# isabella232/kyverno

Measured on AMD Instinct MI355X. Metric: resource×rule validate evals/sec (node), higher is better.
Workload: dtype u8; 1 GPU; C2: synthetic Pods x 100 validate.pattern rules (image globs, ?*, quantities, |-lists); rules=100, pairs_per_gpu=100000000, output=full, parallelism=resource-shard x1, engine=specialized

## Files before the change

### kyverno_amd/csrc/kvapi.cpp

```cpp
#include <hip/hip_runtime.h>
#include <rccl/rccl.h>

#include <chrono>
#include <cstdio>
#include <cstring>

#define KVRT_DEVICE 1
#include "kvrt.hpp"
#include "kvdev.h"

namespace kvh {

struct DevPolicySet {
  DevBuf prog, preds, alts, conjs, atoms, rules, filters, kinds, strrefs, strpairs, sels, sellabels, selexprs, kgs,
      gsegs, gwords, pstr, fword, fbit, flist, frule, rcompact, gsdesc, gsmem;
  uint32_t gs_groups = 0, gs_members = 0;
  DevPS view{};
  std::vector<hipModule_t> mods;
  std::vector<hipFunction_t> fns;
  std::map<uint32_t, std::vector<hipFunction_t>> vfns;
  const std::vector<hipFunction_t>& fns_for(uint32_t full) const {
    auto it = vfns.find(full);
    return it == vfns.end() ? fns : it->second;
  }
// ... 94 lines not shown
    for (const JitImage::Variant& v : J.variants) {
      std::map<std::string, hipFunction_t> vname;
      for (size_t i = 0; i < v.codes.size() && i < J.kernel_name.size(); i++) {
        if (v.codes[i].empty()) continue;
        hipModule_t m;
        HIPCHK(hipModuleLoadData(&m, v.codes[i].data()));
        d->mods.push_back(m);
        hipFunction_t f;
        HIPCHK(hipModuleGetFunction(&f, m, J.kernel_name[i].c_str()));
        vname[J.kernel_name[i]] = f;
      }
      std::vector<hipFunction_t>& fv = d->vfns[v.full];
      for (auto& ch : J.chunks) {
        auto it = vname.find(ch.name);
        fv.push_back(it != vname.end() ? it->second : byname.at(ch.name));
      }
    }
    for (auto& ch : J.chunks) {
      auto it = byname.find(ch.name);
      if (it == byname.end()) throw std::runtime_error("specialized kernel " + ch.name + " missing");
      hipFunction_t f = it->second;
      d->fns.push_back(f);
      if (getenv("KVGPU_VERBOSE")) {
        int regs = 0, local = 0;
        (void)hipFuncGetAttribute(&regs, HIP_FUNC_ATTRIBUTE_NUM_REGS, f);
        (void)hipFuncGetAttribute(&local, HIP_FUNC_ATTRIBUTE_LOCAL_SIZE_BYTES, f);
        fprintf(stderr, "[kvgpu] %s: %zu rules, %d VGPRs, %d B scratch/lane\n", ch.name.c_str(), ch.rules.size(), regs,
                local);
      }
    }
    d->rcompact.upload(J.rec_compact, device);
    if (!J.gs_desc.empty()) {
      d->gs_groups = (uint32_t)(J.gs_desc.size() / 4u);
      d->gs_members = J.gs_members;
      d->gsdesc.upload(J.gs_desc, device);
      d->gsmem.upload(J.gs_mem, device);
    }
    if (J.mtup_words) {
      d->mtup_words = J.mtup_words;
      d->fac_slots = J.fac_slots;
      d->fword.upload(J.fac_word, device);
      d->fbit.upload(J.fac_bit, device);
      d->flist.upload(J.fac_flist, device);
      d->frule.upload(J.fac_rule, device);
      v.fac_word = (const uint32_t*)d->fword.p;
      v.fac_bit = (const uint32_t*)d->fbit.p;
      v.fac_flist = (const uint32_t*)d->flist.p;
      v.fac_rule = (const uint32_t*)d->frule.p;
      v.fac_slots = J.fac_slots;
      v.fac_words = J.mtup_words;
    }
    if (J.memo_words) {
      d->ptab_fn = byname.at("kvj_ptab");
      d->memo_words = J.memo_words;
      d->ptab_rows = (uint32_t)((J.memo_preds.size() + J.ptab_row - 1) / J.ptab_row);
    }
  }
  auto& ref = *d;
  s->dev[device] = std::move(d);
  return ref;
}

void build_pcol(const JitImage& J, const Batch& b, DevBatchRes* d, int device) {
  const auto t0 = std::chrono::steady_clock::now();
  const uint32_t nf = (uint32_t)J.fam_ncols.size(), j0 = J.fam_ncols.at(0);
  const uint64_t groups64 = (b.res.size() + KV_WG - 1) / KV_WG * (KV_WG / KV_LANES);
  if (groups64 > 0x3FFFFFFull) throw std::runtime_error("path columns: too many resources");
  const uint32_t groups = (uint32_t)groups64;
  d->pcold.upload(J.cols, device);
  d->perow.alloc((size_t)std::max<uint32_t>(1u, nf - 1) * (groups + 1) * sizeof(uint32_t), device);
  HIPCHK(hipMemset(d->perow.p, 0, d->perow.n));
  std::vector<ColFam> fams(nf);
  uint32_t n_wide = 0, n_narrow = 0;
  for (uint32_t f = 0; f < nf; f++) {
    fams[f].arr_col = J.fam_arr[f];
    fams[f].ncols = J.fam_ncols[f];
    fams[f].nw = J.fam_nw.at(f);
    fams[f].nb = J.fam_nb.at(f);
    fams[f].nn = J.fam_nn.at(f);
    fams[f].erow = f ? (uint32_t*)d->perow.p + (size_t)(f - 1) * (groups + 1) : nullptr;
    n_wide += fams[f].nw;
    n_narrow += fams[f].nn;
  }
  if (n_narrow && b.vals.size() + KV_PTAB_PSEUDO >= (1ull << KV_COL_PAYLOAD))
    throw std::runtime_error("path columns: more than 2^28 distinct values");
  d->pfam.upload(fams, device);
  const DevBatch* Bd = (const DevBatch*)d->view_dev.p;
  const ColDesc* cd = (const ColDesc*)d->pcold.p;
  std::vector<uint32_t> erow;
  if (nf > 1) {
    HIPCHK(launch_pcol_rows(Bd, cd, (const ColFam*)d->pfam.p, nf, groups, nullptr));
    erow.resize((size_t)(nf - 1) * (groups + 1));
    HIPCHK(hipMemcpy(erow.data(), d->perow.p, erow.size() * sizeof(uint32_t), hipMemcpyDeviceToHost));
  }
  auto row_words = [&](uint32_t f) { return (uint64_t)(3u * fams[f].nw + fams[f].nb + fams[f].nn) * KV_LANES; };
  const uint64_t root_words = (uint64_t)groups * row_words(0);
  uint64_t words = root_words;
  for (uint32_t f = 1; f < nf; f++) {
    fams[f].off_lo = (uint32_t)words;
    fams[f].off_hi = (uint32_t)(words >> 32);
    words += (uint64_t)erow[(size_t)(f - 1) * (groups + 1) + groups] * row_words(f);
  }
  if (words >= (1ull << 32)) throw std::runtime_error("path columns: more than 2^32 words");
  HIPCHK(hipMemcpy(d->pfam.p, fams.data(), fams.size() * sizeof(ColFam), hipMemcpyHostToDevice));
  d->pcol.alloc(std::max<uint64_t>(words, 1) * sizeof(uint32_t), device);
  uint32_t* pool = (uint32_t*)d->pcol.p;
  if (words > root_words) HIPCHK(hipMemset(pool + root_words, 0, (words - root_words) * sizeof(uint32_t)));
  HIPCHK(launch_pcol_build(Bd, cd, (const ColFam*)d->pfam.p, 0, j0, groups, false, pool, nullptr));
  HIPCHK(launch_pcol_build(Bd, cd, (const ColFam*)d->pfam.p, j0, (uint32_t)J.cols.size() - j0, groups, true, pool,
                           nullptr));
  HIPCHK(hipStreamSynchronize(nullptr));
  d->view.pcol = pool;
  d->pcol_ms = std::chrono::duration<double, std::milli>(std::chrono::steady_clock::now() - t0).count();
  if (getenv("KVGPU_VERBOSE"))
    fprintf(stderr,
            "[kvgpu] path columns: %u wide + %u narrow columns in %u families, %llu bytes (%.1f per resource), built in "
            "%.2f ms\n",
            n_wide, n_narrow, nf, (unsigned long long)(words * sizeof(uint32_t)),
            b.res.empty() ? 0.0 : (double)(words * sizeof(uint32_t)) / (double)b.res.size(), d->pcol_ms);
}

std::shared_ptr<DevBatchRes> dev_batch(kv_batch* bt, const PolicySet& ps, int device) {
  std::lock_guard<std::mutex> g(bt->mu);
  auto it = bt->dev.find(device);
  if (it != bt->dev.end()) return it->second;
  auto d = std::make_shared<DevBatchRes>();
  const Batch& b = bt->b;
  if (b.rmask.size() != b.n_rows || b.rwide.size() != b.n_rows || b.roff.size() != b.n_rows)
    throw std::runtime_error("batch: packed row arrays do not match the row count");
  hipStream_t us = StreamPool::get().take(device, hipStreamNonBlocking);
  DevBuf pc, rm, rw, ro;
  pc.upload_async(b.tcells, device, us);
  rm.upload_async(b.rmask, device, us);
  rw.upload_async(b.rwide, device, us);
  ro.upload_async(b.roff, device, us);
  d->vals.upload_async(b.vals, device, us);
  d->nodes.alloc(b.n_cells() * sizeof(Node), device);
  HIPCHK(launch_expand_rows((const uint64_t*)pc.p, (const uint64_t*)rm.p, (const uint64_t*)rw.p, (const uint32_t*)ro.p,
                            (const Val*)d->vals.p, b.n_rows, (Node*)d->nodes.p, us));
  d->res.upload_async(b.res, device, us);
  d->kvs.upload(b.kvs, device);
  d->bstr.upload_raw(b.strs.data(), b.strs.size(), device);
  d->nsbits.upload(b.ns_bits, device);
  std::vector<uint32_t> off, len;
  std::string ks;
  key_table(ps, b, &off, &len, &ks);
  d->koff.upload(off, device);
  d->klen.upload(len, device);
  d->kstr.upload_raw(ks.data(), ks.size(), device);
  d->nsms.upload(b.nsms, device);
  d->lsets.upload(b.lsets, device);
  d->asets.upload(b.asets, device);
  d->tuprep.upload(b.tup_rep, device);
  d->tupkent.upload(b.tup_kent, device);
  d->kentrep.upload(b.kent_rep, device);
  DevBatch& v = d->view;
  v.nodes = (const Node*)d->nodes.p;
  v.vals = (const Val*)d->vals.p;
  v.res = (const Res*)d->res.p;
  v.kvs = (const KV*)d->kvs.p;
  v.bstr = (const uint8_t*)d->bstr.p;
  v.ns_bits = (const uint32_t*)d->nsbits.p;
  v.key_off = (const uint32_t*)d->koff.p;
  v.key_len = (const uint32_t*)d->klen.p;
  v.kstr = (const uint8_t*)d->kstr.p;
  v.nsms = (const StrRef*)d->nsms.p;
  v.lsets = (const KVSet*)d->lsets.p;
  v.asets = (const KVSet*)d->asets.p;
  v.n_nsm = (uint32_t)b.nsms.size();
  v.n_lsets = (uint32_t)b.lsets.size();
  v.n_asets = (uint32_t)b.asets.size();
  v.ns_words = b.ns_words;
  v.n_res = (uint32_t)b.res.size();
  v.tup_rep = (const uint32_t*)d->tuprep.p;
  v.n_tup = (uint32_t)b.tup_rep.size();
  v.tup_kent = (const uint32_t*)d->tupkent.p;
  v.kent_rep = (const uint32_t*)d->kentrep.p;
  v.n_kent = (uint32_t)b.kent_rep.size();
  v.n_ns = (uint32_t)b.namespaces.size();
  {
    const DynHost& h = bt->dyn_host(ps);
    d->dpreds.upload(h.tbl.preds, device);
    d->dalts.upload(h.tbl.alts, device);
    d->dconjs.upload(h.tbl.conjs, device);
    d->datoms.upload(h.tbl.atoms, device);
    d->dgsegs.upload(h.tbl.gsegs, device);
    d->dgwords.upload(h.tbl.gwords, device);
    d->dpstr.upload_raw(h.tbl.strs.data(), h.tbl.strs.size(), device);
    DevPS dv{};
    dv.preds = (const Pred*)d->dpreds.p;
    dv.alts = (const Alt*)d->dalts.p;
    dv.conjs = (const Conj*)d->dconjs.p;
    dv.atoms = (const Atom*)d->datoms.p;
    dv.gsegs = (const GSeg*)d->dgsegs.p;
    dv.gwords = (const GWord*)d->dgwords.p;
    dv.pstr = (const uint8_t*)d->dpstr.p;
    d->dps.upload_raw(&dv, sizeof(DevPS), device);
    d->dleaf.upload(h.dleaf, device);
    d->dynst.upload(h.dyn_st, device);
    v.dps = (const DevPS*)d->dps.p;
    v.dleaf = (const uint32_t*)d->dleaf.p;
    v.dyn_st = (const uint8_t*)d->dynst.p;
  }
  auto up = [&](DevBuf* bufs, std::initializer_list<const std::vector<uint32_t>*> src, const uint32_t** dp) {
    for (const std::vector<uint32_t>* v : src) {
      bufs->alloc(std::max<size_t>(v->size() * sizeof(uint32_t), 16), device);
      if (!v->empty()) HIPCHK(hipMemcpyAsync(bufs->p, v->data(), v->size() * sizeof(uint32_t), hipMemcpyHostToDevice, us));
      *dp++ = (const uint32_t*)(bufs++)->p;
    }
  };
  auto up_blocks = [&](DevBuf* bufs, const CondHost& h, bool strict) {
    const uint32_t* dp[7] = {};
    up(bufs, {&h.sets, &h.ents, &h.outc, &h.truth, &h.unk}, dp);
    if (strict) up(bufs + 5, {&h.err, &h.oos}, dp + 5);
    return CondBlocks{dp[0], dp[1], dp[2], dp[3], dp[4], dp[5], dp[6], h.words};
  };
  struct Timed {
    hipEvent_t e0, e1;
    double* ms;
  };
  std::vector<Timed> timed;
  auto timed_launch = [&](double* ms, auto&& launch) {
    Timed t{nullptr, nullptr, ms};
    HIPCHK(hipEventCreate(&t.e0));
    HIPCHK(hipEventCreate(&t.e1));
    HIPCHK(hipEventRecord(t.e0, us));
    HIPCHK(launch());
    HIPCHK(hipEventRecord(t.e1, us));
    timed.push_back(t);
  };
  CondHost pre, dn;
  FeHost fh;
  CondBlocks pt{}, dt{};
  FeTables ft{};
  const uint32_t n_sets = (uint32_t)ps.csets.size(), n_dsets = (uint32_t)ps.dsets.size(),
                 n_fsets = (uint32_t)ps.fsets.size();
  if (n_sets && !b.res.empty()) {
    build_pre(ps, b, &pre);
    pt = up_blocks(d->pre, pre, false);
    d->prest.alloc((size_t)n_sets * b.res.size(), device);
    v.pre_st = (const uint8_t*)d->prest.p;
  }
  if (n_dsets && !b.res.empty()) {
    build_deny(ps, b, &dn);
    dt = up_blocks(d->dn, dn, true);
  }
  if (n_fsets && !b.res.empty()) {
    build_foreach(ps, b, &fh);
    const uint32_t *dp[5], *gp[2];
    up(d->fe, {&fh.sets, &fh.lists}, dp);
    up(d->feg, {&fh.gate.sets, &fh.gate.ents}, gp);
    ft = fh.view();
    ft.gate = ft.deny = up_blocks(d->fed, fh.deny, true);
    ft.gate.sets = gp[0]; ft.gate.ents = gp[1];
    up(d->fe + 2, {&fh.el_res, &fh.el_ord, &fh.lstate}, dp + 2);
    ft.sets = dp[0]; ft.lists = dp[1]; ft.el_res = dp[2]; ft.el_ord = dp[3]; ft.lstate = dp[4];
    d->feacc.alloc((size_t)n_fsets * b.res.size() * sizeof(uint32_t), device);
  }
  if ((n_dsets || n_fsets) && !b.res.empty()) {
    d->dnst.alloc((size_t)(n_dsets + n_fsets) * b.res.size(), device);
    v.deny_st = (const uint8_t*)d->dnst.p;
  }
  d->view_dev.upload_raw(&d->view, sizeof(DevBatch), device);
  if (v.pre_st) timed_launch(&d->pre_ms, [&]() { return launch_cond(false, pt, v.n_res, n_sets, (uint8_t*)d->prest.p, us); });
  if (v.deny_st && n_dsets)
    timed_launch(&d->deny_ms, [&]() { return launch_cond(true, dt, v.n_res, n_dsets, (uint8_t*)d->dnst.p, us); });
  if (v.deny_st && n_fsets)
    timed_launch(&d->fe_ms, [&]() {
      return launch_foreach(ft, v.n_res, (uint32_t*)d->feacc.p, (uint8_t*)d->dnst.p + (size_t)n_dsets * v.n_res, us);
    });
  HIPCHK(hipStreamSynchronize(us));
  for (const Timed& t : timed) {
    float ms = 0;
    HIPCHK(hipEventElapsedTime(&ms, t.e0, t.e1));
    *t.ms = ms;
    (void)hipEventDestroy(t.e0);
    (void)hipEventDestroy(t.e1);
  }
  StreamPool::get().give(device, hipStreamNonBlocking, us);
  pc.release();
  rm.release();
  rw.release();
  ro.release();
  if (bt->owner && bt->owner->jit && !bt->owner->jit->cols.empty() && !b.res.empty()) {
    build_pcol(*bt->owner->jit, b, d.get(), device);
    d->view_dev.upload_raw(&d->view, sizeof(DevBatch), device);
  }
  bt->dev[device] = d;
  return d;
}

struct DevSession {
  kv_policyset* ps = nullptr;
  kv_batch* bt = nullptr;
  int device = 0;
  uint32_t mode = 0;
  uint64_t nrules = 0, nres = 0;
  DevBuf fflags, pview, st, er8, er, cn, scope, scn, ptab, mtab, mtbf, mtup, ftab;
  DevBuf ptab1, pview1, mtab1, mtup1, ftab1, cn1, scn1;
  uint32_t *mt1_ns = nullptr, *mt1_ann = nullptr, *mt1_sel = nullptr;
  hipStream_t pside = nullptr;
  hipEvent_t ev_pt[2] = {nullptr, nullptr}, ev_rk[2] = {nullptr, nullptr};
  bool ptab_pipe = false;
  uint32_t fac_entities = 0, ntup = 0;
  bool rec_compact = false;
  std::shared_ptr<DevBatchRes> batch_ref;
  DevBuf r_offs, r_tot, r_base, r_out8, r_outw, r_wide;
  DevBuf r_tkey, r_raw, r_nbase, r_code, r_out8b;
  DevBuf s_ccnt, s_cbase, s_pack;
  HostArray<uint8_t> hstage;
  DevBuf inv_d, stc;
  DevBuf ord_d, r_mask;
  DevBuf stamps;
  DevBuf gsite, gcnt;
  DevBuf sflag;
  uint32_t mt_words = 0, mt_entities = 0;
  uint32_t *mt_ns = nullptr, *mt_ann = nullptr, *mt_sel = nullptr;
  uint32_t nscopes = 0, nvals = 0;
  DevOut O{};
  const DevBatch* bview = nullptr;
  const DevBatch* bhost = nullptr;
  DevPolicySet* dps = nullptr;
  hipStream_t stream = nullptr;
  hipEvent_t e0 = nullptr, e1 = nullptr;
  hipStream_t side = nullptr;
  hipEvent_t ev_fork = nullptr, ev_join = nullptr;
  hipEvent_t ev_rkf = nullptr, ev_rkj[3] = {};
  std::vector<hipStream_t> rkx;
  std::vector<hipEvent_t> kev;
  std::vector<uint32_t> korder;
  bool ktiming = false;

  double upload_ms = 0;
  DevSession(kv_policyset* p, kv_batch* b, const char* ctx_json, int dev, uint32_t m)
      : ps(p), bt(b), device(dev), mode(m) {
    HIPCHK(hipSetDevice(device));
    const auto tc0 = std::chrono::steady_clock::now();
    DevPolicySet& dp = dev_ps(ps, device);
    batch_ref = dev_batch(bt, ps->ps, device);
    DevBatchRes& db = *batch_ref;
    upload_ms = std::chrono::duration<double, std::milli>(std::chrono::steady_clock::now() - tc0).count();
    if (getenv("KVGPU_VERBOSE")) fprintf(stderr, "[kvgpu] session: policy set + batch upload %.1f ms\n", upload_ms);
    bview = (const DevBatch*)db.view_dev.p;
    bhost = &db.view;
    dps = &dp;
    fflags.upload(fold_filters(ps->ps, ctx_json), device);
    DevPS P = dp.view;
    P.fflags = (const uint32_t*)fflags.p;
    if (dp.ptab_fn) {
      nvals = (uint32_t)bt->b.vals.size();
      ptab.alloc((size_t)dp.memo_words * (nvals + KV_PTAB_PSEUDO) * sizeof(uint32_t), device);
      P.ptab = (const uint32_t*)ptab.p;
      P.n_vals = nvals + KV_PTAB_PSEUDO;
    }
    {
      const PolicySet& pp = ps->ps;
      const Batch& bb = bt->b;
      P.mt_ns_words = (pp.n_nss_bits + 31) / 32;
      P.mt_ann_words = (pp.n_ann_bits + 31) / 32;
      P.mt_sel_words = (uint32_t)((pp.selectors.size() + 31) / 32);
      const size_t n_ns = (size_t)P.mt_ns_words * bb.nsms.size(), n_an = (size_t)P.mt_ann_words * bb.asets.size(),
                   n_sl = (size_t)P.mt_sel_words * bb.lsets.size();
      mtab.alloc(std::max<size_t>(n_ns + n_an + n_sl, 1) * sizeof(uint32_t), device);
      mt_ns = (uint32_t*)mtab.p;
      mt_ann = mt_ns + n_ns;
      mt_sel = mt_ann + n_an;
      P.mt_ns = mt_ns;
      P.mt_ann = mt_ann;
      mtbf.upload(mtab_bit_filters(pp), device);
      P.mt_bitf = (const uint32_t*)mtbf.p;
      P.mt_sel = mt_sel;
      mt_words = P.mt_ns_words + P.mt_ann_words + P.mt_sel_words;
      mt_entities = (uint32_t)std::max({bb.nsms.size(), bb.asets.size(), bb.lsets.size()});
    }
    if (dp.mtup_words) {
      mtup.alloc(std::max<size_t>((size_t)dp.mtup_words * bt->b.tup_rep.size(), 1) * sizeof(uint32_t), device);
      P.mtup = (const uint32_t*)mtup.p;
      P.mtup_words = dp.mtup_words;
      const DevBatch& bv = *bhost;
      const uint32_t ne[KV_FAC_TYPES] = {bv.n_kent, bv.n_nsm, bv.n_asets, bv.n_lsets, bv.n_ns};
      uint64_t at = 0;
      for (uint32_t t = 0; t < KV_FAC_TYPES; t++) {
        P.fac_off[t] = at;
        at += (uint64_t)dp.fac_slots * ne[t];
        fac_entities = std::max(fac_entities, ne[t]);
      }
      ftab.alloc(std::max<uint64_t>(at, 1) * sizeof(uint32_t), device);
      P.fac_tab = (uint32_t*)ftab.p;
    }
    pview.upload_raw(&P, sizeof(DevPS), device);
    ptab_pipe = dp.specialized() && !(getenv("KVGPU_PTAB_PIPE") && getenv("KVGPU_PTAB_PIPE")[0] == '0');
    if (ptab_pipe) {
      if (dp.ptab_fn) {
        ptab1.alloc(ptab.n, device);
        P.ptab = (const uint32_t*)ptab1.p;
      }
      mtab1.alloc(mtab.n, device);
      mt1_ns = (uint32_t*)mtab1.p;
      mt1_ann = mt1_ns + (mt_ann - mt_ns);
      mt1_sel = mt1_ns + (mt_sel - mt_ns);
      P.mt_ns = mt1_ns;
      P.mt_ann = mt1_ann;
      P.mt_sel = mt1_sel;
      if (dp.mtup_words) {
        mtup1.alloc(mtup.n, device);
        P.mtup = (const uint32_t*)mtup1.p;
        ftab1.alloc(ftab.n, device);
        P.fac_tab = (uint32_t*)ftab1.p;
      }
      pview1.upload_raw(&P, sizeof(DevPS), device);
    }
    nrules = ps->ps.rules.size();
    nres = bt->b.res.size();
    ntup = (uint32_t)bt->b.tup_rep.size();
    O.full = 0;
    if ((mode & (KV_MODE_STATUS | KV_MODE_ERRORS)) || ((mode & KV_MODE_SCOPES) && !dp.specialized())) {
      st.alloc(nrules * nres, device);
      O.status = (uint8_t*)st.p;
      O.full |= 1;
      if (dp.specialized()) {
        sflag.alloc(std::max<uint64_t>(nrules * ((nres + KV_RWG - 1) / KV_RWG), 1), device);
        HIPCHK(hipMemset(sflag.p, 1, sflag.n));
        O.sflag = (uint8_t*)sflag.p;
      }
    }
    if (mode & KV_MODE_ERRORS) {
      er8.alloc(nrules * nres * sizeof(ErrRec8), device);
      O.err8 = (ErrRec8*)er8.p;
      O.err = nullptr;
      O.full |= 2;
      if (dp.gs_groups) {
        const uint64_t nw = (nres + 63) / 64;
        gsite.alloc(std::max<uint64_t>((uint64_t)dp.gs_members * nw * 64u * 16u, 16), device);
        gcnt.alloc(std::max<uint64_t>((uint64_t)dp.gs_groups * nw * sizeof(uint32_t), 4), device);
        O.gsite = (uint32_t*)gsite.p;
        O.gcnt = (uint32_t*)gcnt.p;
      }
    }
    cn.alloc(std::max<uint64_t>(nrules, 1) * KV_HIST * sizeof(unsigned long long), device);
    O.counts = (unsigned long long*)cn.p;
    if (ptab_pipe) cn1.alloc(cn.n, device);
    if (mode & KV_MODE_SCOPES) {
      std::vector<uint32_t> sc(nres);
      for (uint64_t i = 0; i < nres; i++) sc[i] = bt->b.res[i].ns_index;
      nscopes = (uint32_t)bt->b.namespaces.size();
      scope.upload(sc, device);
      scn.alloc(std::max<uint64_t>((uint64_t)nscopes * nrules, 1) * KV_HIST * sizeof(unsigned long long), device);
      if (ptab_pipe) scn1.alloc(scn.n, device);
      O.scope = (const uint32_t*)scope.p;
      O.scounts = (unsigned long long*)scn.p;
      if (dp.specialized()) O.full |= 8;
    }
    if (getenv("KVGPU_JIT_STAMPS") && dp.specialized()) {
      const uint64_t n = (nres + KV_RWG - 1) / KV_RWG * KV_RWAVES * kJitStamps;
      stamps.alloc(std::max<uint64_t>(n, 1) * sizeof(unsigned long long), device);
      HIPCHK(hipMemset(stamps.p, 0, stamps.n));
      for (hipModule_t m : dp.mods) {
        hipDeviceptr_t g = nullptr;
        size_t gs = 0;
        if (hipModuleGetGlobal(&g, &gs, m, "kvj_stamps") == hipSuccess && gs == sizeof(void*))
          HIPCHK(hipMemcpy(g, &stamps.p, sizeof(void*), hipMemcpyHostToDevice));
        else
          (void)hipGetLastError();
      }
    }
    stream = StreamPool::get().take(device, hipStreamDefault);
    HIPCHK(hipEventCreate(&e0));
    HIPCHK(hipEventCreate(&e1));
    side = StreamPool::get().take(device, hipStreamNonBlocking);
    if (ptab_pipe) {
      pside = StreamPool::get().take(device, hipStreamNonBlocking, true);
      for (int b = 0; b < 2; b++) {
        HIPCHK(hipEventCreateWithFlags(&ev_pt[b], hipEventDisableTiming));
        HIPCHK(hipEventCreateWithFlags(&ev_rk[b], hipEventDisableTiming));
      }
    }
    HIPCHK(hipEventCreateWithFlags(&ev_fork, hipEventDisableTiming));
    HIPCHK(hipEventCreateWithFlags(&ev_join, hipEventDisableTiming));
    HIPCHK(hipEventCreateWithFlags(&ev_rkf, hipEventDisableTiming));
    for (hipEvent_t& e : ev_rkj) HIPCHK(hipEventCreateWithFlags(&e, hipEventDisableTiming));
  }
  void detach_batch() { bt = nullptr; }
  void remap_scopes(const std::vector<uint32_t>& map, uint32_t n_total) {
    if (!(mode & KV_MODE_SCOPES)) return;
    HIPCHK(hipSetDevice(device));
    DevBuf m;
    m.upload(map, device);
    HIPCHK(launch_remap_u32((uint32_t*)scope.p, nres, (const uint32_t*)m.p, stream));
    HIPCHK(hipStreamSynchronize(stream));
    nscopes = n_total;
    scn.alloc(std::max<uint64_t>((uint64_t)nscopes * nrules, 1) * KV_HIST * sizeof(unsigned long long), device);
    if (ptab_pipe) scn1.alloc(scn.n, device);
    O.scounts = (unsigned long long*)scn.p;
  }
  ~DevSession() {
    (void)hipSetDevice(device);
    if (e0) (void)hipEventDestroy(e0);
    if (e1) (void)hipEventDestroy(e1);
    if (ev_fork) (void)hipEventDestroy(ev_fork);
    if (ev_join) (void)hipEventDestroy(ev_join);
    if (ev_rkf) (void)hipEventDestroy(ev_rkf);
    for (hipEvent_t e : ev_rkj)
      if (e) (void)hipEventDestroy(e);
    for (hipEvent_t e : kev) (void)hipEventDestroy(e);
    for (hipStream_t x : rkx) StreamPool::get().give(device, hipStreamNonBlocking, x);
    for (int b = 0; b < 2; b++) {
      if (ev_pt[b]) (void)hipEventDestroy(ev_pt[b]);
      if (ev_rk[b]) (void)hipEventDestroy(ev_rk[b]);
    }
    StreamPool::get().give(device, hipStreamNonBlocking, pside, true);
    StreamPool::get().give(device, hipStreamNonBlocking, side);
    StreamPool::get().give(device, hipStreamDefault, stream);
  }
  double run(int iters, bool vm = false) {
    HIPCHK(hipSetDevice(device));
    HIPCHK(hipEventRecord(e0, stream));
    const bool pipe = ptab_pipe && dps->specialized() && !vm && nres;
    if (pipe && iters > 0) {
      HIPCHK(hipStreamWaitEvent(pside, e0, 0));
      launch_tables(0);
    }
    for (int i = 0; i < iters; i++) {
      rec_compact = dps->specialized() && !vm;
      if (pipe) {
        const int b = i & 1;
        launch_specialized(b);
        if (O.full & 8u)
          HIPCHK(launch_scope_totals((const unsigned long long*)(b ? scn1.p : scn.p), nscopes, (uint32_t)nrules,
                                     (unsigned long long*)(b ? cn1.p : cn.p), stream));
        HIPCHK(hipEventRecord(ev_rk[b], stream));
        if (i + 1 < iters) {
          const int nb = (i + 1) & 1;
          if (i >= 1) HIPCHK(hipStreamWaitEvent(pside, ev_rk[nb], 0));
          launch_tables(nb);
        }
        continue;
      }
      hipStream_t ms = rec_compact ? side : stream;
      if (rec_compact) {
        HIPCHK(hipEventRecord(ev_fork, stream));
        HIPCHK(hipStreamWaitEvent(side, ev_fork, 0));
      }
      HIPCHK(hipMemsetAsync(cn.p, 0, cn.n, ms));
      if (mode & KV_MODE_SCOPES) HIPCHK(hipMemsetAsync(scn.p, 0, scn.n, ms));
      HIPCHK(launch_mtab((const DevPS*)pview.p, bview, mt_words, mt_entities, mt_ns, mt_ann, mt_sel, ms));
      if (rec_compact) {
        launch_specialized();
        if (O.full & 8u)
          HIPCHK(launch_scope_totals((const unsigned long long*)scn.p, nscopes, (uint32_t)nrules,
                                     (unsigned long long*)cn.p, stream));
      } else {
        DevOut Ov = O;
        Ov.full &= ~8u;
        HIPCHK(launch_validate((const DevPS*)pview.p, bview, (uint32_t)nres, Ov, 0, (uint32_t)nrules, stream));
        if (mode & KV_MODE_SCOPES)
          HIPCHK(launch_scope_counts(O.status, (const uint32_t*)scope.p, (uint32_t)nres, (uint32_t)nrules, nscopes,
                                     (unsigned long long*)scn.p, stream));
      }
    }
    HIPCHK(hipEventRecord(e1, stream));
    HIPCHK(hipEventSynchronize(e1));
    order_kernels();
    if (pipe && iters > 0 && ((iters - 1) & 1)) {
      cn.swap(cn1);
      scn.swap(scn1);
      O.counts = (unsigned long long*)cn.p;
      if (mode & KV_MODE_SCOPES) O.scounts = (unsigned long long*)scn.p;
    }
    float t = 0;
    HIPCHK(hipEventElapsedTime(&t, e0, e1));
    if (stamps.p) report_stamps();
    return t;
  }
  void report_stamps() {
    std::vector<unsigned long long> h(stamps.n / sizeof(unsigned long long));
    HIPCHK(hipMemcpy(h.data(), stamps.p, stamps.n, hipMemcpyDeviceToHost));
    double seg[kJitStamps] = {}, life = 0;
    uint64_t n[kJitStamps] = {}, nl = 0;
    for (size_t w = 0; w + kJitStamps <= h.size(); w += kJitStamps) {
      const unsigned long long* x = &h[w];
      uint32_t last = 0;
      for (uint32_t k = 1; k < kJitStamps; k++)
        if (x[k] && x[last]) {
          seg[k] += (double)(x[k] - x[last]);
          n[k]++;
          last = k;
        }
      if (x[0] && x[last] && last) {
        life += (double)(x[last] - x[0]);
        nl++;
      }
    }
    fprintf(stderr, "[kvgpu] stamps: wave lifetime %.0f cycles;", nl ? life / nl : 0.0);
    for (uint32_t k = 1; k < kJitStamps; k++)
      if (n[k]) fprintf(stderr, " seg%u %.0f", k, seg[k] / n[k]);
    fprintf(stderr, "\n");
  }
  void launch_tables(int b) {
    const DevPS* P = (const DevPS*)(b ? pview1.p : pview.p);
    DevBuf& c = b ? cn1 : cn;
    HIPCHK(hipMemsetAsync(c.p, 0, c.n, pside));
    if (mode & KV_MODE_SCOPES) {
      DevBuf& sc = b ? scn1 : scn;
      HIPCHK(hipMemsetAsync(sc.p, 0, sc.n, pside));
    }
    HIPCHK(launch_mtab(P, bview, mt_words, mt_entities, b ? mt1_ns : mt_ns, b ? mt1_ann : mt_ann, b ? mt1_sel : mt_sel,
                       pside));
    if (dps->mtup_words && ntup)
      HIPCHK(launch_mfac(P, bview, dps->fac_slots, fac_entities, dps->mtup_words, ntup,
                         (uint32_t*)(b ? mtup1.p : mtup.p), pside));
    if (dps->ptab_fn) {
      const Val* V = bhost->vals;
      const uint8_t* S = bhost->bstr;
      uint32_t NV = nvals;
      uint32_t* PT = (uint32_t*)(b ? ptab1.p : ptab.p);
      void* targs[] = {(void*)&P, (void*)&V, (void*)&S, (void*)&NV, (void*)&PT};
      HIPCHK(hipModuleLaunchKernel(dps->ptab_fn, (NV + KV_PTAB_PSEUDO + KV_WG - 1) / KV_WG, dps->ptab_rows, 1, KV_WG, 1, 1,
                                   0, pside, targs, nullptr));
    }
    HIPCHK(hipEventRecord(ev_pt[b], pside));
  }
  void launch_specialized(int pb = -1) {
    if (nres == 0) {
      HIPCHK(hipEventRecord(ev_join, side));
      HIPCHK(hipStreamWaitEvent(stream, ev_join, 0));
      return;
    }
    const uint32_t blocks = (uint32_t)((nres + KV_RWG - 1) / KV_RWG);
    const DevPS* P = (const DevPS*)(pb == 1 ? pview1.p : pview.p);
    const Node* N = bhost->nodes;
    const Val* V = bhost->vals;
    const uint8_t* S = bhost->bstr;
    if (pb >= 0) {
      HIPCHK(hipStreamWaitEvent(stream, ev_pt[pb], 0));
    } else {
    if (dps->ptab_fn) {
      uint32_t NV = nvals;
      uint32_t* PT = (uint32_t*)ptab.p;
      void* targs[] = {(void*)&P, (void*)&V, (void*)&S, (void*)&NV, (void*)&PT};
      HIPCHK(hipModuleLaunchKernel(dps->ptab_fn, (NV + KV_PTAB_PSEUDO + KV_WG - 1) / KV_WG, dps->ptab_rows, 1, KV_WG, 1, 1, 0,
                                   stream, targs, nullptr));
    }
    if (dps->mtup_words && ntup)
      HIPCHK(launch_mfac(P, bview, dps->fac_slots, fac_entities, dps->mtup_words, ntup, (uint32_t*)mtup.p, side));
    HIPCHK(hipEventRecord(ev_join, side));
    HIPCHK(hipStreamWaitEvent(stream, ev_join, 0));
    }
    DevOut Ov = O;
    if (pb == 1) {
      Ov.counts = (unsigned long long*)cn1.p;
      if (mode & KV_MODE_SCOPES) Ov.scounts = (unsigned long long*)scn1.p;
    }
    uint32_t r0 = 0;
    void* args[] = {(void*)&P, (void*)&bview, (void*)&N, (void*)&V, (void*)&S, (void*)&Ov, (void*)&r0};
    constexpr uint32_t kRuleStreams = 3;
    const std::vector<hipFunction_t>& fs = dps->fns_for(Ov.full);
    const uint32_t nk = (uint32_t)fs.size();
    if (korder.empty() && nk > 1) {
      std::lock_guard<std::mutex> g(dps->order_mu);
      if (dps->korder.size() == nk) korder = dps->korder;
    }
    const bool ordered = korder.size() == nk && nk > 1;
    const uint32_t ns = nk >= 3 ? std::min<uint32_t>(kRuleStreams, nk) : (ordered ? nk : 1u);
    const bool timing = !ordered && nk > 1 && !ktiming;
    if (timing) {
      while (kev.size() < 2 * nk) {
        hipEvent_t e;
        HIPCHK(hipEventCreate(&e));
        kev.push_back(e);
      }
      ktiming = true;
    }
    while (rkx.size() + 2 < ns) rkx.push_back(StreamPool::get().take(device, hipStreamNonBlocking));
    hipStream_t sts[4] = {stream, side, rkx.size() > 0 ? rkx[0] : nullptr, rkx.size() > 1 ? rkx[1] : nullptr};
    if (ns > 1) {
      HIPCHK(hipEventRecord(ev_rkf, stream));
      for (uint32_t q = 1; q < ns; q++) HIPCHK(hipStreamWaitEvent(sts[q], ev_rkf, 0));
    }
    for (uint32_t k = 0; k < nk; k++) {
      const uint32_t f = ordered ? korder[k] : k;
      hipStream_t st = sts[k % ns];
      if (timing) HIPCHK(hipEventRecord(kev[2 * f], st));
      HIPCHK(hipModuleLaunchKernel(fs[f], blocks, 1, 1, KV_RWG, 1, 1, 0, st, args, nullptr));
      if (timing) HIPCHK(hipEventRecord(kev[2 * f + 1], st));
    }
    for (uint32_t q = 1; q < ns; q++) {
      HIPCHK(hipEventRecord(ev_rkj[q - 1], sts[q]));
      HIPCHK(hipStreamWaitEvent(stream, ev_rkj[q - 1], 0));
    }
  }
  void order_kernels() {
    if (!ktiming || !korder.empty()) return;
    const uint32_t nk = (uint32_t)(kev.size() / 2);
    std::vector<std::pair<float, uint32_t>> d(nk);
    for (uint32_t k = 0; k < nk; k++) {
      float ms = 0.f;
      if (hipEventElapsedTime(&ms, kev[2 * k], kev[2 * k + 1]) != hipSuccess) {
        (void)hipGetLastError();
        return;
      }
      d[k] = {ms, k};
    }
    std::stable_sort(d.begin(), d.end(), [](const auto& a, const auto& b) { return a.first > b.first; });
    for (const auto& x : d) korder.push_back(x.second);
    std::lock_guard<std::mutex> g(dps->order_mu);
    if (dps->korder.empty()) dps->korder = korder;
  }
  uint64_t written_status_bytes() {
    if (!O.status) return 0;
    if (!O.sflag || !dps->specialized()) return nrules * nres;
    HIPCHK(hipSetDevice(device));
    HIPCHK(hipStreamSynchronize(stream));
    std::vector<uint8_t> f(sflag.n);
    if (!f.empty()) HIPCHK(hipMemcpy(f.data(), sflag.p, f.size(), hipMemcpyDeviceToHost));
    const uint64_t nwg = (nres + KV_RWG - 1) / KV_RWG, last = nres - (nwg - 1) * KV_RWG;
    uint64_t bytes = 0;
    for (uint64_t i = 0; i < nrules * nwg && i < f.size(); i++)
      if (f[i]) bytes += (i % nwg == nwg - 1) ? last : KV_RWG;
    return bytes;
  }
  std::vector<int64_t> read_counts() {
    HIPCHK(hipSetDevice(device));
    std::vector<unsigned long long> c(nrules * KV_HIST);
    if (!c.empty()) HIPCHK(hipMemcpy(c.data(), cn.p, c.size() * sizeof(unsigned long long), hipMemcpyDeviceToHost));
    return std::vector<int64_t>(c.begin(), c.end());
  }
  std::vector<int64_t> read_scope_counts() {
    HIPCHK(hipSetDevice(device));
    std::vector<unsigned long long> c((size_t)nscopes * nrules * KV_HIST);
    if (!c.empty()) HIPCHK(hipMemcpy(c.data(), scn.p, c.size() * sizeof(unsigned long long), hipMemcpyDeviceToHost));
    return std::vector<int64_t>(c.begin(), c.end());
  }
  void fetch(kv_result* out, ResultPart* part, uint64_t lo, uint64_t n_total) {
    HIPCHK(hipSetDevice(device));
    const bool verbose = getenv("KVGPU_VERBOSE") != nullptr;
    auto tl = std::chrono::steady_clock::now();
    auto lap = [&](const char* what) {
      HIPCHK(hipStreamSynchronize(stream));
      const auto now = std::chrono::steady_clock::now();
      const double ms = std::chrono::duration<double, std::milli>(now - tl).count();
      tl = now;
      if (part == &out->parts[0]) out->phases.push_back({what, ms});
      if (verbose) fprintf(stderr, "[kvgpu] fetch: %s %.1f ms\n", what, ms);
    };
    const bool want_st = O.status && (mode & (KV_MODE_STATUS | KV_MODE_ERRORS)) && nres && nrules;
    bool side_copy = false;
    uint64_t spack_bytes = 0;
    const bool packed = want_st && out->sparse;
    if (packed) {
      const uint64_t nwg = (nres + KV_RWG - 1) / KV_RWG, nch = (nwg + KV_WG - 1) / KV_WG;
      if (s_ccnt.n < nrules * nch * sizeof(uint32_t)) {
        s_ccnt.alloc(nrules * nch * sizeof(uint32_t), device);
        s_cbase.alloc(nrules * nch * sizeof(unsigned long long), device);
      }
      HIPCHK(launch_status_pack(O.status, O.sflag, (uint32_t)nres, (uint32_t)nrules, nullptr, (uint32_t*)s_ccnt.p,
                                nullptr, stream));
      std::vector<uint32_t> cc(nrules * nch);
      std::vector<unsigned long long> cb(nrules * nch);
      HIPCHK(hipMemcpyAsync(cc.data(), s_ccnt.p, cc.size() * sizeof(uint32_t), hipMemcpyDeviceToHost, stream));
      HIPCHK(hipStreamSynchronize(stream));
      part->nwg = nwg;
      part->sbase.resize(nrules);
      unsigned long long t = 0;
      for (size_t i = 0; i < cc.size(); i++) {
        if (i % nch == 0) part->sbase[i / nch] = t;
        cb[i] = t;
        t += cc[i];
      }
      const uint64_t bytes = t * (KV_RWG / 2);
      if (s_pack.n < std::max<uint64_t>(bytes, 1)) s_pack.alloc(std::max<uint64_t>(bytes, 1), device);
      HIPCHK(hipMemcpyAsync(s_cbase.p, cb.data(), cb.size() * sizeof(unsigned long long), hipMemcpyHostToDevice, stream));
      HIPCHK(launch_status_pack(O.status, O.sflag, (uint32_t)nres, (uint32_t)nrules,
                                (const unsigned long long*)s_cbase.p, nullptr, (uint8_t*)s_pack.p, stream));
      part->sflag.alloc(nrules * nwg);
      part->spack.alloc(bytes);
      spack_bytes = bytes;
      lap("status_pack");
    }
    bool caller = !packed && want_st && bt && lo == 0 && nres == n_total && !bt->b.order.empty();
    if (caller && !stc.p) {
      size_t fr = 0, tot = 0;
      if (hipMemGetInfo(&fr, &tot) != hipSuccess) caller = false;
      fr += dev_pool_held(device);
      if (fr < nrules * nres + nres * 8u + (512ull << 20)) caller = false;
    }
    if (caller) {
      if (!inv_d.p) inv_d.upload_raw(bt->inverse(), nres * sizeof(uint32_t), device);
      if (!stc.p) stc.alloc(nrules * nres, device);
      HIPCHK(launch_gather_rows((const uint8_t*)st.p, (const uint32_t*)inv_d.p, nrules, nres, (uint8_t*)stc.p, stream));
      HIPCHK(hipEventRecord(ev_fork, stream));
      HIPCHK(hipStreamWaitEvent(side, ev_fork, 0));
      HIPCHK(hipMemcpyAsync(out->status.data(), stc.p, nrules * nres, hipMemcpyDeviceToHost, side));
      side_copy = true;
      out->caller_order = true;
      lap("status_gather");
    } else if (want_st && !packed) {
      HIPCHK(hipMemcpy2DAsync(out->status.data() + lo, n_total, st.p, nres, nres, nrules, hipMemcpyDeviceToHost,
                              stream));
      lap("status_d2h");
    }
    if (O.err8 && nres && nrules) {
      const uint32_t tiles = (uint32_t)((nres + KV_WG - 1) / KV_WG);
      part->tiles = tiles;
      if (!r_offs.p) {
        r_offs.alloc((size_t)nrules * tiles * sizeof(uint32_t), device);
        r_tot.alloc(nrules * sizeof(unsigned long long), device);
        r_base.alloc((nrules + 1) * sizeof(unsigned long long), device);
        r_wide.alloc(sizeof(uint32_t), device);
      }
      const uint32_t* ord = nullptr;
      unsigned long long* masks = nullptr;
      if (caller) {
        if (!ord_d.p) ord_d.upload_raw(bt->b.order.data(), nres * sizeof(uint32_t), device);
        if (!r_mask.p) r_mask.alloc((size_t)nrules * tiles * (KV_WG / 64) * sizeof(unsigned long long), device);
        ord = (const uint32_t*)ord_d.p;
        masks = (unsigned long long*)r_mask.p;
      }
      const uint8_t* rank_st = caller ? (const uint8_t*)stc.p : O.status;
      const uint8_t* seg_flags = rec_compact && !caller ? O.sflag : nullptr;
      HIPCHK(launch_rec_compact(rank_st, O.err8, nullptr, (uint32_t)nres, (uint32_t)nrules, (uint32_t*)r_offs.p,
                                (unsigned long long*)r_tot.p, (unsigned long long*)r_base.p, nullptr, nullptr, nullptr,
                                0, rec_compact ? (const uint8_t*)dps->rcompact.p : nullptr, nullptr, masks, seg_flags,
                                stream));
      const size_t tb = (size_t)nrules * KV_REC_CODES, sb = ((nrules + 1) * 8 + 63) & ~(size_t)63;
      if (hstage.size() < sb + nrules * 4 + 64 + tb * 8) hstage.alloc(sb + nrules * 4 + 64 + tb * 8);
      part->base.resize(nrules + 1);
      part->offs.alloc((size_t)nrules * tiles);
      HIPCHK(hipMemcpyAsync(hstage.data(), r_base.p, part->base.size() * sizeof(uint64_t), hipMemcpyDeviceToHost, stream));
      HIPCHK(hipMemcpyAsync(part->offs.data(), r_offs.p, part->offs.size() * sizeof(uint32_t), hipMemcpyDeviceToHost,
                            stream));
      lap("records_count");
      memcpy(part->base.data(), hstage.data(), part->base.size() * sizeof(uint64_t));
      const uint64_t total = part->base[nrules];
      if (r_out8.n < total * sizeof(ErrRec8)) {
        r_out8.alloc(std::max<uint64_t>(total, 1) * sizeof(ErrRec8), device);
        lap("records_alloc");
      }
      HIPCHK(hipMemsetAsync(r_wide.p, 0, sizeof(uint32_t), stream));
      if (rec_compact && O.gsite) {
        HIPCHK(launch_gsite_expand(O.gsite, O.gcnt, (const GSiteDesc*)dps->gsdesc.p, (const uint32_t*)dps->gsmem.p,
                                   dps->gs_groups, (uint32_t)nres, O.err8, stream));
        lap("records_expand");
      }
      HIPCHK(launch_rec_compact(O.status, O.err8, nullptr, (uint32_t)nres, (uint32_t)nrules, (uint32_t*)r_offs.p,
                                nullptr, (unsigned long long*)r_base.p, (ErrRec8*)r_out8.p, nullptr,
                                (uint32_t*)r_wide.p, 1, rec_compact ? (const uint8_t*)dps->rcompact.p : nullptr, ord,
                                masks, seg_flags, stream));
      HIPCHK(hipMemcpyAsync(hstage.data() + sb, r_wide.p, sizeof(uint32_t), hipMemcpyDeviceToHost, stream));
      lap("records_scatter");
      uint32_t wide = 0;
      memcpy(&wide, hstage.data() + sb, sizeof(uint32_t));
      const ErrRec8* src = (const ErrRec8*)r_out8.p;
      uint64_t keep = total;
      bool coded = false;
      part->raw.clear();
      if (!wide && total && nrules) {
        if (r_tkey.n < tb * sizeof(unsigned long long)) {
          r_tkey.alloc(tb * sizeof(unsigned long long), device);
          r_raw.alloc(nrules * sizeof(uint32_t), device);
          r_nbase.alloc(nrules * sizeof(unsigned long long), device);
        }
        if (r_code.n < total) r_code.alloc(total, device);
        HIPCHK(hipMemsetAsync(r_tkey.p, 0xFF, tb * sizeof(unsigned long long), stream));
        HIPCHK(hipMemsetAsync(r_raw.p, 0, nrules * sizeof(uint32_t), stream));
        HIPCHK(launch_rec_codes((const ErrRec8*)r_out8.p, (const unsigned long long*)r_base.p, (uint32_t)nrules,
                                (unsigned long long*)r_tkey.p, (uint8_t*)r_code.p, (uint32_t*)r_raw.p, nullptr, nullptr,
                                0, stream));
        const uint32_t* rawf = (const uint32_t*)hstage.data();
        const unsigned long long* keys = (const unsigned long long*)(hstage.data() + ((nrules * 4 + 63) & ~(size_t)63));
        HIPCHK(hipMemcpyAsync((void*)rawf, r_raw.p, nrules * sizeof(uint32_t), hipMemcpyDeviceToHost, stream));
        HIPCHK(hipMemcpyAsync((void*)keys, r_tkey.p, tb * sizeof(unsigned long long), hipMemcpyDeviceToHost, stream));
        HIPCHK(hipStreamSynchronize(stream));
        part->raw.assign(nrules, 0);
        part->nbase.assign(nrules, 0);
        part->tab.assign(tb, ErrRec8{0u, 0u});
        keep = 0;
        for (uint64_t q = 0; q < nrules; q++) {
          part->raw[q] = rawf[q] ? 1 : 0;
          part->nbase[q] = keep;
          if (rawf[q]) keep += part->base[q + 1] - part->base[q];
        }
        for (size_t t = 0; t < tb; t++)
          if (keys[t] != ~0ull) part->tab[t] = ErrRec8{(uint32_t)(keys[t] >> 32), (uint32_t)keys[t]};
        if (keep) {
          if (r_out8b.n < keep * sizeof(ErrRec8)) r_out8b.alloc(keep * sizeof(ErrRec8), device);
          HIPCHK(hipMemcpyAsync(r_nbase.p, part->nbase.data(), nrules * sizeof(unsigned long long),
                                hipMemcpyHostToDevice, stream));
          HIPCHK(launch_rec_codes((const ErrRec8*)r_out8.p, (const unsigned long long*)r_base.p, (uint32_t)nrules,
                                  nullptr, nullptr, (uint32_t*)r_raw.p, (const unsigned long long*)r_nbase.p,
                                  (ErrRec8*)r_out8b.p, 1, stream));
          src = (const ErrRec8*)r_out8b.p;
        }
        coded = true;
        lap("records_code");
      }
      const auto th0 = std::chrono::steady_clock::now();
      part->rec.alloc(keep);
      if (part == &out->parts[0])
        out->phases.push_back(
            {"host_alloc", std::chrono::duration<double, std::milli>(std::chrono::steady_clock::now() - th0).count()});
      if (coded) part->code.alloc(total);
      tl = std::chrono::steady_clock::now();
      if (keep) HIPCHK(hipMemcpyAsync(part->rec.data(), src, keep * sizeof(ErrRec8), hipMemcpyDeviceToHost, stream));
      if (coded) HIPCHK(hipMemcpyAsync(part->code.data(), r_code.p, total, hipMemcpyDeviceToHost, stream));
      lap("records_d2h");
      if (wide) {
        if (!er.p) er.alloc(nrules * nres * sizeof(ErrRec), device);
        O.err = (ErrRec*)er.p;
        O.full |= 4;
        run(1, true);
        O.full &= ~4u;
        if (r_outw.n < total * sizeof(ErrRec)) r_outw.alloc(std::max<uint64_t>(total, 1) * sizeof(ErrRec), device);
        HIPCHK(launch_rec_compact(O.status, O.err8, O.err, (uint32_t)nres, (uint32_t)nrules, (uint32_t*)r_offs.p,
                                  nullptr, (unsigned long long*)r_base.p, (ErrRec8*)r_out8.p, (ErrRec*)r_outw.p,
                                  (uint32_t*)r_wide.p, 1, nullptr, ord, masks, nullptr, stream));
        part->recw.alloc(total);
        HIPCHK(hipMemcpyAsync(part->recw.data(), r_outw.p, total * sizeof(ErrRec), hipMemcpyDeviceToHost, stream));
        lap("records_wide_rerun");
      }
    }
    if (packed) {
      HIPCHK(hipMemcpyAsync(part->sflag.data(), O.sflag, part->sflag.size(), hipMemcpyDeviceToHost, stream));
      if (spack_bytes) HIPCHK(hipMemcpyAsync(part->spack.data(), s_pack.p, spack_bytes, hipMemcpyDeviceToHost, stream));
      lap("status_d2h");
    }
    HIPCHK(hipStreamSynchronize(stream));
    if (side_copy) {
      HIPCHK(hipStreamSynchronize(side));
      lap("status_d2h_wait");
    }
  }
};

struct SessionSet {
  kv_policyset* ps = nullptr;
  kv_batch* bt = nullptr;
  uint32_t mode = 0;
  uint64_t nrules = 0, nres = 0;
  std::vector<std::shared_ptr<kv_batch>> shards;
  std::vector<std::pair<uint64_t, uint64_t>> ranges;
  std::vector<std::unique_ptr<DevSession>> parts;
  std::vector<ncclComm_t> comms;
  bool reduced = false;
  std::vector<int64_t> counts_, scope_counts_;
  std::vector<double> part_ms;
  bool parts_mode = false, finalized = true;
  std::string ctx;
  std::vector<int> devs;
  std::vector<std::vector<std::string>> part_ns;
  std::vector<std::string> scope_names;

  SessionSet(kv_policyset* p, const char* ctx_json, uint32_t m, uint32_t n)
      : ps(p), mode(m), parts_mode(true), finalized(false), ctx(ctx_json ? ctx_json : "") {
    nrules = ps->ps.rules.size();
    parts.resize(n);
    ranges.assign(n, {0, 0});
    devs.assign(n, -1);
    part_ns.resize(n);
  }
  void attach(uint32_t k, kv_batch* b, int d) {
    if (!parts_mode || finalized) throw std::runtime_error("not an open parts session");
    if (k >= parts.size()) throw std::runtime_error("part index out of range");
    if (parts[k]) throw std::runtime_error("part already attached");
    auto ds = std::make_unique<DevSession>(ps, b, ctx.empty() ? nullptr : ctx.c_str(), d, mode);
    part_ns[k] = b->b.namespaces;
    ds->detach_batch();
    parts[k] = std::move(ds);
    devs[k] = d;
    for (auto& q : parts)
      if (!q) return;
    finalize();
  }
  void finalize() {
    uint64_t at = 0;
    for (size_t k = 0; k < parts.size(); k++) {
      ranges[k] = {at, at + parts[k]->nres};
      at += parts[k]->nres;
// ... 589 lines not shown
```

Measured before the change: 293.7 billion evals/s.

## Double-buffer output arrays so consecutive validate passes overlap on two streams

Allocates a second set of per-pair output buffers (status, sflag, err8, gsite, gcnt) and runs odd iterations of the specialized validate kernel on the side stream, writing into that second set. Consecutive passes can then run concurrently instead of serializing on one stream. The buffers are swapped after the run so the caller sees the last pass's results. The path is taken only when there is a single kernel, enough free memory for the extra set, and no stamp tracing. It costs a duplicate full-output allocation and adds contention between the two concurrent passes.

```diff
diff --git a/kyverno_amd/csrc/kvapi.cpp b/kyverno_amd/csrc/kvapi.cpp
--- a/kyverno_amd/csrc/kvapi.cpp
+++ b/kyverno_amd/csrc/kvapi.cpp
@@ -420,6 +420,9 @@
   hipStream_t pside = nullptr;
   hipEvent_t ev_pt[2] = {nullptr, nullptr}, ev_rk[2] = {nullptr, nullptr};
   bool ptab_pipe = false;
+  DevBuf st1, er81, sflag1, gsite1, gcnt1;
+  bool pass_overlap = false;
+  int set1 = -1;
   uint32_t fac_entities = 0, ntup = 0;
   bool rec_compact = false;
   std::shared_ptr<DevBatchRes> batch_ref;
@@ -508,6 +511,7 @@
     }
     pview.upload_raw(&P, sizeof(DevPS), device);
     ptab_pipe = dp.specialized() && !(getenv("KVGPU_PTAB_PIPE") && getenv("KVGPU_PTAB_PIPE")[0] == '0');
+    pass_overlap = ptab_pipe && !(getenv("KVGPU_PASS_OVERLAP") && getenv("KVGPU_PASS_OVERLAP")[0] == '0');
     if (ptab_pipe) {
       if (dp.ptab_fn) {
         ptab1.alloc(ptab.n, device);
@@ -632,8 +636,10 @@
   }
   double run(int iters, bool vm = false) {
     HIPCHK(hipSetDevice(device));
+    const bool pipe = ptab_pipe && dps->specialized() && !vm && nres;
+    const bool ov =
+        pipe && pass_overlap && iters >= 2 && !stamps.p && dps->fns_for(O.full).size() == 1 && second_set();
     HIPCHK(hipEventRecord(e0, stream));
-    const bool pipe = ptab_pipe && dps->specialized() && !vm && nres;
     if (pipe && iters > 0) {
       HIPCHK(hipStreamWaitEvent(pside, e0, 0));
       launch_tables(0);
@@ -642,11 +648,12 @@
       rec_compact = dps->specialized() && !vm;
       if (pipe) {
         const int b = i & 1;
-        launch_specialized(b);
+        hipStream_t xs = ov && b ? side : stream;
+        launch_specialized(b, ov);
         if (O.full & 8u)
           HIPCHK(launch_scope_totals((const unsigned long long*)(b ? scn1.p : scn.p), nscopes, (uint32_t)nrules,
-                                     (unsigned long long*)(b ? cn1.p : cn.p), stream));
-        HIPCHK(hipEventRecord(ev_rk[b], stream));
+                                     (unsigned long long*)(b ? cn1.p : cn.p), xs));
+        HIPCHK(hipEventRecord(ev_rk[b], xs));
         if (i + 1 < iters) {
           const int nb = (i + 1) & 1;
           if (i >= 1) HIPCHK(hipStreamWaitEvent(pside, ev_rk[nb], 0));
@@ -676,6 +683,7 @@
                                      (unsigned long long*)scn.p, stream));
       }
     }
+    if (ov) HIPCHK(hipStreamWaitEvent(stream, ev_rk[1], 0));
     HIPCHK(hipEventRecord(e1, stream));
     HIPCHK(hipEventSynchronize(e1));
     order_kernels();
@@ -684,11 +692,59 @@
       scn.swap(scn1);
       O.counts = (unsigned long long*)cn.p;
       if (mode & KV_MODE_SCOPES) O.scounts = (unsigned long long*)scn.p;
+      if (ov) {
+        st.swap(st1);
+        sflag.swap(sflag1);
+        er8.swap(er81);
+        gsite.swap(gsite1);
+        gcnt.swap(gcnt1);
+        if (O.status) O.status = (uint8_t*)st.p;
+        if (O.sflag) O.sflag = (uint8_t*)sflag.p;
+        if (O.err8) O.err8 = (ErrRec8*)er8.p;
+        if (O.gsite) O.gsite = (uint32_t*)gsite.p;
+        if (O.gcnt) O.gcnt = (uint32_t*)gcnt.p;
+      }
     }
     float t = 0;
     HIPCHK(hipEventElapsedTime(&t, e0, e1));
     if (stamps.p) report_stamps();
     return t;
+  }
+  bool second_set() {
+    if (set1 < 0) set1 = take_second_set() ? 1 : 0;
+    return set1 == 1;
+  }
+  bool take_second_set() {
+    const size_t need = st.n + sflag.n + er8.n + gsite.n + gcnt.n;
+    if (!need) return true;
+    const bool verbose = getenv("KVGPU_VERBOSE") != nullptr;
+    if (const char* e = getenv("KVGPU_PASS_OVERLAP_MAX_BYTES"))
+      if (need > strtoull(e, nullptr, 10)) {
+        if (verbose) fprintf(stderr, "[kvgpu] session: second output set %.1f MB over the cap, passes in order\n", need / 1e6);
+        return false;
+      }
+    size_t fr = 0, tot = 0;
+    if (hipMemGetInfo(&fr, &tot) != hipSuccess) {
+      (void)hipGetLastError();
+      return false;
+    }
+    if (fr + dev_pool_held(device) < 2 * need + (1ull << 30)) return false;
+    try {
+      if (st.p) st1.alloc(st.n, device);
+      if (sflag.p) {
+        sflag1.alloc(sflag.n, device);
+        HIPCHK(hipMemset(sflag1.p, 1, sflag1.n));
+      }
+      if (er8.p) er81.alloc(er8.n, device);
+      if (gsite.p) gsite1.alloc(gsite.n, device);
+      if (gcnt.p) gcnt1.alloc(gcnt.n, device);
+    } catch (const HipError&) {
+      (void)hipGetLastError();
+      for (DevBuf* x : {&st1, &sflag1, &er81, &gsite1, &gcnt1}) x->release();
+      return false;
+    }
+    if (verbose) fprintf(stderr, "[kvgpu] session: second output set %.1f MB\n", need / 1e6);
+    return true;
   }
   void report_stamps() {
     std::vector<unsigned long long> h(stamps.n / sizeof(unsigned long long));
@@ -738,7 +794,7 @@
     }
     HIPCHK(hipEventRecord(ev_pt[b], pside));
   }
-  void launch_specialized(int pb = -1) {
+  void launch_specialized(int pb = -1, bool ov = false) {
     if (nres == 0) {
       HIPCHK(hipEventRecord(ev_join, side));
       HIPCHK(hipStreamWaitEvent(stream, ev_join, 0));
@@ -749,8 +805,9 @@
     const Node* N = bhost->nodes;
     const Val* V = bhost->vals;
     const uint8_t* S = bhost->bstr;
+    hipStream_t xs = ov && pb == 1 ? side : stream;
     if (pb >= 0) {
-      HIPCHK(hipStreamWaitEvent(stream, ev_pt[pb], 0));
+      HIPCHK(hipStreamWaitEvent(xs, ev_pt[pb], 0));
     } else {
     if (dps->ptab_fn) {
       uint32_t NV = nvals;
@@ -768,6 +825,13 @@
     if (pb == 1) {
       Ov.counts = (unsigned long long*)cn1.p;
       if (mode & KV_MODE_SCOPES) Ov.scounts = (unsigned long long*)scn1.p;
+      if (ov) {
+        if (O.status) Ov.status = (uint8_t*)st1.p;
+        if (O.sflag) Ov.sflag = (uint8_t*)sflag1.p;
+        if (O.err8) Ov.err8 = (ErrRec8*)er81.p;
+        if (O.gsite) Ov.gsite = (uint32_t*)gsite1.p;
+        if (O.gcnt) Ov.gcnt = (uint32_t*)gcnt1.p;
+      }
     }
     uint32_t r0 = 0;
     void* args[] = {(void*)&P, (void*)&bview, (void*)&N, (void*)&V, (void*)&S, (void*)&Ov, (void*)&r0};
@@ -790,7 +854,7 @@
       ktiming = true;
     }
     while (rkx.size() + 2 < ns) rkx.push_back(StreamPool::get().take(device, hipStreamNonBlocking));
-    hipStream_t sts[4] = {stream, side, rkx.size() > 0 ? rkx[0] : nullptr, rkx.size() > 1 ? rkx[1] : nullptr};
+    hipStream_t sts[4] = {xs, side, rkx.size() > 0 ? rkx[0] : nullptr, rkx.size() > 1 ? rkx[1] : nullptr};
     if (ns > 1) {
       HIPCHK(hipEventRecord(ev_rkf, stream));
       for (uint32_t q = 1; q < ns; q++) HIPCHK(hipStreamWaitEvent(sts[q], ev_rkf, 0));
```

Measured after the change: 304.2 billion evals/s, median of 6. +3.6%, better.
